# cboin1996/avddpg

Hardware: NVIDIA B200
Metric: platoon-vehicle env-steps/s (higher is better)
Workload: dtype fp16

## Files before the change

### avddpg_b200/csrc/avd_fused3.cu

```cuda
#include <cudaTypedefs.h>

#include <algorithm>

#include "avd_common.cuh"
#include "avd_ddpg_layout.cuh"
#include "avd_umma.cuh"

namespace avd {
namespace fused3 {

using namespace umma;
typedef __nv_bfloat16 bf16;

constexpr int TILE_M = 128, L2N = 128, KB = 64, MAX_KB = 5, L1N = 256;
constexpr int NCONS = 16;
constexpr int NUM_THREADS = 32 * (1 + NCONS);
constexpr int SLOT_BYTES = TILE_M * KB * 2;
constexpr int MAX_SLOT = 7;
constexpr int OFF_W = 0;
constexpr int OFF_RING = OFF_W + MAX_KB * SLOT_BYTES;
constexpr int OFF_DZ = OFF_RING + 5 * SLOT_BYTES;
constexpr int OFF_B1 = OFF_RING + MAX_SLOT * SLOT_BYTES;
constexpr int B1_BYTES = 2 * L1N * 16;
constexpr int OFF_X = OFF_B1 + B1_BYTES;
constexpr int X_BYTES = 2 * TILE_M * 16;
constexpr int OFF_TAB = OFF_X + 2 * X_BYTES;
constexpr int TAB_BYTES = 2048;
constexpr int OFF_PART = OFF_TAB + TAB_BYTES;
constexpr int OFF_BAR = OFF_PART + 2 * 4 * TILE_M * 4;
constexpr int SMEM_BYTES = OFF_BAR + 512 + 1024;
constexpr int kVRows = 49, kVStride = 132, kVBrk = 64;
static_assert((kVRows * kVStride + kVBrk) * 4 + 2 * 4 * TILE_M * 4 <= 2 * SLOT_BYTES, "V table + partial sums exceed the dz2-tile slots");
static_assert(SMEM_BYTES <= 232448, "exceeds the 227 KB shared memory of an sm_100 CTA");

enum Mode { MODE_ACTOR_OUT = 0, MODE_TARGET = 1, MODE_Q = 2, MODE_CRITIC_BWD = 3, MODE_ACTOR_BWD = 4, MODE_CRITIC_ACTION = 5, MODE_ACTOR_SAVE = 6 };

struct Args {
    avd_net_dims d;
    int A;
    int64_t R;
    const float* params;
    int64_t pstride;
    const float* b2f;
    const float* s;
    int64_t s_rs, s_cs;
    const float* act;
    const float* rew;
    float gamma, high;
    const float* y;
    const float* dpi;
    float* out;
    uint32_t* mask_out;
    int mask_words;
    uint32_t* mask2_out;
    float* dact_out;
    const float* vtab;
    float dm_scale;
    float* sdq;
    float* loss;
    int tiles_per_agent, ctas_per_agent;
};

__device__ __forceinline__ uint32_t pack_bf16x2(float a, float b) {
    __nv_bfloat162 v = __floats2bfloat162_rn(a, b);
    return *reinterpret_cast<uint32_t*>(&v);
}
__device__ __forceinline__ uint32_t pack_f16x2(float a, float b) {
    __half2 v = __floats2half2_rn(a, b);
    return *reinterpret_cast<uint32_t*>(&v);
}
__device__ __forceinline__ uint64_t make_desc_noswz(uint32_t saddr, uint32_t lbo_bytes, uint32_t sbo_bytes) {
    return (uint64_t)((saddr & 0x3FFFFu) >> 4) | ((uint64_t)((lbo_bytes >> 4) & 0x3FFFu) << 16) |
           ((uint64_t)((sbo_bytes >> 4) & 0x3FFFu) << 32) | (1ull << 46);
}
__device__ __forceinline__ void split_bf16(float v, bf16& hi, bf16& lo) {
    hi = __float2bfloat16_rn(v);
    lo = __float2bfloat16_rn(v - __bfloat162float(hi));
}
__device__ __forceinline__ uint32_t pack2(bf16 a, bf16 b) {
    return (uint32_t)__bfloat16_as_ushort(a) | ((uint32_t)__bfloat16_as_ushort(b) << 16);
}

template <int MODE, bool F16>
__global__ void __launch_bounds__(NUM_THREADS, 1) fused3_kernel(const __grid_constant__ CUtensorMap tmW, const __grid_constant__ CUtensorMap tmDZ, Args g) {
    constexpr bool CRITIC = MODE != MODE_ACTOR_OUT && MODE != MODE_ACTOR_BWD && MODE != MODE_ACTOR_SAVE;
    constexpr bool SAVE = MODE == MODE_ACTOR_SAVE;
    constexpr bool BWD = MODE == MODE_CRITIC_BWD || MODE == MODE_ACTOR_BWD;
    constexpr bool ACTION = MODE == MODE_CRITIC_ACTION;
    constexpr bool HAS_DZ = BWD;
    constexpr int NKB = CRITIC ? 5 : 4;
    constexpr int NSLOT = (HAS_DZ || ACTION) ? 5 : MAX_SLOT;
    constexpr uint32_t FOP = F16 ? FMT_F16 : FMT_BF16;

    extern __shared__ uint8_t smem_raw[];
    uint8_t* smem = smem_raw + ((1024u - (smem_u32(smem_raw) & 1023u)) & 1023u);
    float* b2f_tab = reinterpret_cast<float*>(smem + OFF_TAB);
    float* w3f_tab = b2f_tab + L2N;
    float* wa_tab = w3f_tab + L2N;
    float* ba_tab = wa_tab + 64;
    float* scal = ba_tab + 64;
    float* part = reinterpret_cast<float*>(smem + OFF_PART);
    uint64_t* a_full = reinterpret_cast<uint64_t*>(smem + OFF_BAR);
    uint64_t* a_empty = a_full + MAX_SLOT;
    uint64_t* acc_full = a_empty + MAX_SLOT;
    uint64_t* acc_empty = acc_full + 2;
    uint64_t* part_full = acc_empty + 2;
    uint64_t* x_full = part_full + 2;
    uint64_t* z1_full = x_full + 2;
    uint64_t* z1_empty = z1_full + 1;
    uint64_t* dz_full = z1_empty + 1;
    uint64_t* dz_empty = dz_full + 1;
    uint64_t* dra_full = dz_empty + 1;
    uint64_t* dra_empty = dra_full + 1;
    uint64_t* w_full = dra_empty + 1;
    uint32_t* tmem_slot = reinterpret_cast<uint32_t*>(w_full + 1);

    const int warp = threadIdx.x >> 5, lane = threadIdx.x & 31;
    const avd_net_dims d = g.d;
    const int la = CRITIC ? d.la : 0;
    const int agent = (int)blockIdx.x / g.ctas_per_agent;
    const int cta = (int)blockIdx.x - agent * g.ctas_per_agent;
    const int T = (g.tiles_per_agent - cta + g.ctas_per_agent - 1) / g.ctas_per_agent;
    const float* P = g.params + (int64_t)agent * g.pstride;

    if (threadIdx.x == 0) {
        tma_prefetch_desc(&tmW);
        if (BWD) tma_prefetch_desc(&tmDZ);
        for (int i = 0; i < MAX_SLOT; ++i) { mbar_init(&a_full[i], 8); mbar_init(&a_empty[i], 1); }
        for (int i = 0; i < 2; ++i) {
            mbar_init(&acc_full[i], 1); mbar_init(&acc_empty[i], NCONS);
            mbar_init(&part_full[i], NCONS); mbar_init(&x_full[i], 4);
        }
        mbar_init(z1_full, 1); mbar_init(z1_empty, NCONS);
        mbar_init(dz_full, NCONS); mbar_init(dz_empty, 1);
        mbar_init(dra_full, 1); mbar_init(dra_empty, 4);
        mbar_init(w_full, 1);
        fence_barrier_init();
    }
    if (warp == 0) tmem_alloc(tmem_slot, 512);

    if (warp >= 1) {
        const int ct = threadIdx.x - 32;
        int64_t oW, ob, og2, obe2, omu2, ovar2, oW3, ob3;
        if (CRITIC) { const CriticOff o = critic_off(d); oW = o.Ws; ob = o.bs; og2 = o.g2; obe2 = o.be2; omu2 = o.mu2; ovar2 = o.var2; oW3 = o.W3; ob3 = o.b3; }
        else { const ActorOff o = actor_off(d); oW = o.W1; ob = o.b1; og2 = o.g2; obe2 = o.be2; omu2 = o.mu2; ovar2 = o.var2; oW3 = o.W3; ob3 = o.b3; }
        if (ct < L1N) {
            bf16 whi[4], wlo[4], bhi, blo;
#pragma unroll
            for (int k = 0; k < 4; ++k) split_bf16(k < d.ns ? P[oW + (int64_t)k * d.l1 + ct] : 0.0f, whi[k], wlo[k]);
            split_bf16(P[ob + ct], bhi, blo);
            const bf16 zero = __float2bfloat16_rn(0.0f);
            const uint4 c0 = make_uint4(pack2(whi[0], whi[1]), pack2(whi[2], whi[3]), pack2(bhi, whi[0]), pack2(whi[1], whi[2]));
            const uint4 c1 = make_uint4(pack2(whi[3], bhi), pack2(wlo[0], wlo[1]), pack2(wlo[2], wlo[3]), pack2(blo, zero));
            *reinterpret_cast<uint4*>(smem + OFF_B1 + ct * 16) = c0;
            *reinterpret_cast<uint4*>(smem + OFF_B1 + L1N * 16 + ct * 16) = c1;
        } else if (ct < L1N + L2N) {
            const int c = ct - L1N;
            const float sc2 = P[og2 + c] / sqrtf(P[ovar2 + c] + kBnEps);
            const float sh2 = P[obe2 + c] - P[omu2 + c] * sc2;
            const float w3 = P[oW3 + c];
            w3f_tab[c] = w3 * sc2;
            const float t = warp_sum(sh2 * w3);
            if (lane == 0) scal[1 + (c >> 5)] = t;
            if (c == 0) scal[5] = P[ob3];
        } else if (ct < L1N + L2N + 64) {
            const int c = ct - L1N - L2N;
            float wa = 0.f, ba = 0.f;
            if (CRITIC && c < d.la) { const CriticOff o = critic_off(d); wa = P[o.Wa + c]; ba = P[o.ba + c]; }
            wa_tab[c] = wa;
            ba_tab[c] = ba;
        }
        fence_proxy_async();
    }
    tc_fence_before();
    __syncthreads();
    tc_fence_after();
    const uint32_t tmem_base = *tmem_slot;
    pdl_wait();
    pdl_launch_dependents();
    if (threadIdx.x >= 32 && threadIdx.x < 32 + L2N) b2f_tab[threadIdx.x - 32] = g.b2f[(int64_t)agent * L2N + threadIdx.x - 32];
    float* vtab_s = reinterpret_cast<float*>(smem + OFF_DZ);
    float* vbrk_s = vtab_s + kVRows * kVStride;
    float* part2 = vbrk_s + kVBrk;
    if (ACTION) {
        const float4* src = reinterpret_cast<const float4*>(g.vtab + (int64_t)agent * (kVRows * kVStride + kVBrk));
        for (int i = threadIdx.x; i < (kVRows * kVStride + kVBrk) / 4; i += NUM_THREADS) reinterpret_cast<float4*>(vtab_s)[i] = src[i];
    }
    __syncthreads();
    const float b3f = scal[5] + scal[1] + scal[2] + scal[3] + scal[4];
    if (T <= 0) {
        __syncthreads();
        if (warp == 0) tmem_dealloc(tmem_base, 512);
        return;
    }

    auto tile_of = [&](int tc) { return cta + tc * g.ctas_per_agent; };

    if (warp == 0) {
        {
            const uint32_t leader = elect_one();
            constexpr uint32_t idesc1 = make_idesc_bf16(TILE_M, L2N, false, false);
            constexpr uint32_t idesc = make_idesc_f16kind(TILE_M, L2N, false, false, FOP, FOP);
            const int F = L1N + la;
            const uint64_t dW = make_smem_desc(smem_u32(smem + OFF_W), 16, 1024);
            const uint64_t dR = make_smem_desc(smem_u32(smem + OFF_RING), 16, 1024);
            const uint64_t dX = make_desc_noswz(smem_u32(smem + OFF_X), TILE_M * 16, 128);
            const uint64_t dB1 = make_desc_noswz(smem_u32(smem + OFF_B1), L1N * 16, 128);
            mbar_expect_tx_p(leader, w_full, (uint32_t)NKB * SLOT_BYTES);
            for (int kb = 0; kb < NKB; ++kb) tma_load_3d_p(leader, smem + OFF_W + kb * SLOT_BYTES, &tmW, w_full, kb * KB, 0, agent);

            auto mma1 = [&](int t) {
                mbar_wait(&x_full[t & 1], ((uint32_t)t >> 1) & 1);
                if (t >= 1) mbar_wait(z1_empty, (uint32_t)(t - 1) & 1);
                tc_fence_after();
#pragma unroll
                for (int h = 0; h < 2; ++h)
                    mma_bf16_p(leader, tmem_base + 256u + (uint32_t)(h * L2N), desc_add(dX, (uint32_t)(t & 1) * X_BYTES), desc_add(dB1, h * (L2N * 16)), idesc1, 0);
                mma_commit_p(leader, z1_full);
            };
            auto mma2 = [&](int t) {
                mbar_wait(&acc_empty[t & 1], (((uint32_t)t >> 1) & 1) ^ 1);
                tc_fence_after();
                const uint32_t tacc = tmem_base + (uint32_t)((t & 1) * L2N);
#pragma unroll
                for (int kb = 0; kb < NKB; ++kb) {
                    const uint32_t kc = (uint32_t)(t * NKB + kb), sl = kc % NSLOT;
                    mbar_wait(&a_full[sl], (kc / NSLOT) & 1);
                    tc_fence_after();
                    const int nm = min(4, (F - kb * KB) / 16);
#pragma unroll
                    for (int j = 0; j < 4; ++j)
                        if (j < nm)
                            mma_bf16_p(leader, tacc, desc_add(dR, sl * SLOT_BYTES + j * 32), desc_add(dW, kb * SLOT_BYTES + j * 32), idesc, (kb | j) != 0);
                    mma_commit_p(leader, &a_empty[sl]);
                }
                mma_commit_p(leader, &acc_full[t & 1]);
            };
            auto dz_out = [&](int t) {
                mbar_wait(dz_full, (uint32_t)t & 1);
                tc_fence_after();
                tma_store_3d_p(leader, &tmDZ, smem + OFF_DZ, 0, tile_of(t) * TILE_M, agent);
                tma_store_3d_p(leader, &tmDZ, smem + OFF_DZ + SLOT_BYTES, KB, tile_of(t) * TILE_M, agent);
                if (leader) {
                    bulk_commit();
                    bulk_wait_read0();
                }
                __syncwarp();
                mbar_arrive_p(leader, dz_empty);
            };

            mbar_wait(w_full, 0);
            {
                mma1(0);
                if (T > 1) mma1(1);
                mma2(0);
                for (int i = 0; i < T; ++i) {
                    if (i + 1 < T) {
                        if (i + 2 < T) mma1(i + 2);
                        mma2(i + 1);
                    }
                    if (BWD && i >= 1) dz_out(i - 1);
                }
                if (BWD) dz_out(T - 1);
            }
        }
    } else {
        const int cw = warp - 1;
        const int q = warp & 3;
        const int c4 = cw >> 2;
        const int row = q * 32 + lane;
        const uint32_t tlane = (uint32_t)(q * 32) << 16;
        const float invR = 1.0f / (float)g.R;
        float sdq_acc = 0.0f, loss_acc = 0.0f;
        uint32_t zneg = 0u;

        auto rowinfo = [&](int tc, bool& valid) -> int64_t {
            const int64_t r_in = (int64_t)tile_of(tc) * TILE_M + row;
            valid = r_in < g.R;
            return (int64_t)agent * g.R + (valid ? r_in : g.R - 1);
        };
        float xs[4] = {0.f, 0.f, 0.f, 0.f}, a_pf = 0.0f, y_pf = 0.0f, a_ag = 0.0f;
        auto xg_of = [&](int tc) { return CRITIC ? 2 * (1 - (tc & 1)) : (tc & 3); };
        auto is_action_quarter = [&](int tc) { return CRITIC && (c4 >> 1) == (tc & 1); };
        auto load_x = [&](int t) {
            bool valid;
            const int64_t n = rowinfo(t, valid);
#pragma unroll
            for (int k = 0; k < 4; ++k) xs[k] = k < d.ns ? __ldg(g.s + n * g.s_rs + k * g.s_cs) : 0.0f;
        };
        auto write_x = [&](int t) {
            bf16 hi[5], lo[5];
#pragma unroll
            for (int k = 0; k < 4; ++k) split_bf16(xs[k], hi[k], lo[k]);
            hi[4] = __float2bfloat16_rn(1.0f);
            lo[4] = __float2bfloat16_rn(0.0f);
            uint8_t* xbase = smem + OFF_X + (t & 1) * X_BYTES;
            *reinterpret_cast<uint4*>(xbase + row * 16) = make_uint4(pack2(hi[0], hi[1]), pack2(hi[2], hi[3]), pack2(hi[4], lo[0]), pack2(lo[1], lo[2]));
            *reinterpret_cast<uint4*>(xbase + TILE_M * 16 + row * 16) =
                make_uint4(pack2(lo[3], lo[4]), pack2(hi[0], hi[1]), pack2(hi[2], hi[3]), pack2(hi[4], lo[4]));
            fence_proxy_async();
            __syncwarp();
            if (lane == 0) mbar_arrive(&x_full[t & 1]);
        };

        auto convert = [&](int tc) {
            bool valid;
            const int64_t nrow = rowinfo(tc, valid);
            const int ga0 = CRITIC ? 2 * (tc & 1) : -1;
            const float a_val = a_pf;
            mbar_wait(z1_full, (uint32_t)tc & 1);
            tc_fence_after();
            const uint32_t kc = (uint32_t)(tc * NKB + c4), sl = kc % NSLOT;
            mbar_wait(&a_empty[sl], ((kc / NSLOT) & 1) ^ 1);
            uint8_t* slot = smem + OFF_RING + sl * SLOT_BYTES + row * 128;
            uint32_t neg[2];
#pragma unroll
            for (int h = 0; h < 2; ++h) {
                float z[32];
                tmem_ld32(tmem_base + 256u + (uint32_t)(c4 * 64 + h * 32) + tlane, z);
                uint32_t m = 0;
                if (BWD || SAVE) {
#pragma unroll
                    for (int j = 0; j < 32; ++j) m = __funnelshift_l(__float_as_uint(z[j]), m, 1);
                }
                neg[h] = m;
#pragma unroll
                for (int k = 0; k < 4; ++k) {
                    const uint4 pk = make_uint4(pack_relu_x2<F16>(z[8 * k], z[8 * k + 1]), pack_relu_x2<F16>(z[8 * k + 2], z[8 * k + 3]),
                                                pack_relu_x2<F16>(z[8 * k + 4], z[8 * k + 5]), pack_relu_x2<F16>(z[8 * k + 6], z[8 * k + 7]));
                    *reinterpret_cast<uint4*>(slot + (((h * 4 + k) ^ (row & 7)) << 4)) = pk;
                }
            }
            tc_fence_before();
            fence_proxy_async();
            __syncwarp();
            if (lane == 0) { mbar_arrive(z1_empty); mbar_arrive_cnt(&a_full[sl], 2); }
            if ((BWD || SAVE) && valid) *reinterpret_cast<uint2*>(g.mask_out + nrow * g.mask_words + 2 * c4) = make_uint2(neg[0], neg[1]);
            if (CRITIC && (c4 == ga0 || c4 == ga0 + 1)) {
                const int j0 = (c4 == ga0) ? 0 : 32;
                const uint32_t kca = (uint32_t)(tc * NKB + 4), sla = kca % NSLOT;
                mbar_wait(&a_empty[sla], ((kca / NSLOT) & 1) ^ 1);
                uint8_t* aslot = smem + OFF_RING + sla * SLOT_BYTES + row * 128;
                float z[32];
                uint32_t m = 0;
#pragma unroll
                for (int j = 0; j < 32; ++j) {
                    z[j] = fmaf(a_val, wa_tab[j0 + j], ba_tab[j0 + j]);
                    if (BWD) m = __funnelshift_l(__float_as_uint(z[j]), m, 1);
                }
#pragma unroll
                for (int k = 0; k < 4; ++k) {
                    const int col = j0 + 8 * k;
                    if (col < la) {
                        const uint4 pk = make_uint4(pack_relu_x2<F16>(z[8 * k], z[8 * k + 1]), pack_relu_x2<F16>(z[8 * k + 2], z[8 * k + 3]),
                                                    pack_relu_x2<F16>(z[8 * k + 4], z[8 * k + 5]), pack_relu_x2<F16>(z[8 * k + 6], z[8 * k + 7]));
                        *reinterpret_cast<uint4*>(aslot + (((col >> 3) ^ (row & 7)) << 4)) = pk;
                    }
                }
                fence_proxy_async();
                __syncwarp();
                if (lane == 0) mbar_arrive(&a_full[sla]);
                if (BWD && valid) g.mask_out[nrow * g.mask_words + 8 + (j0 >> 5)] = m;
            }
            if (c4 == xg_of(tc) && tc + 2 < T) write_x(tc + 2);
            if (tc + 3 < T && c4 == xg_of(tc + 1)) load_x(tc + 3);
            if (tc + 1 < T && is_action_quarter(tc + 1)) {
                bool v1;
                a_pf = __ldg(g.act + rowinfo(tc + 1, v1));
            }
        };

        auto pass1 = [&](int tc) {
            const int buf = tc & 1;
            if (MODE == MODE_TARGET || BWD) {
                bool v0;
                const int64_t n0 = rowinfo(tc, v0);
                if (MODE == MODE_TARGET) { if (c4 == 0) y_pf = __ldg(g.rew + n0); }
                else if (MODE == MODE_CRITIC_BWD) y_pf = __ldg(g.y + n0);
                else y_pf = __ldg(g.dpi + n0);
            }
            const float* vrow = vtab_s;
            if (ACTION) {
                const float a_cur = a_ag;
                if (tc + 1 < T) {
                    bool v1;
                    a_ag = __ldg(g.act + rowinfo(tc + 1, v1));
                }
                int k = 0;
#pragma unroll
                for (int st = 32; st >= 1; st >>= 1)
                    if (vbrk_s[k + st - 1] < a_cur) k += st;
                vrow = vtab_s + k * kVStride + c4 * 32;
            }
            mbar_wait(&acc_full[buf], ((uint32_t)tc >> 1) & 1);
            tc_fence_after();
            float v[32];
            tmem_ld32(tmem_base + (uint32_t)(buf * L2N + c4 * 32) + tlane, v);
            float acc = 0.0f, gacc = 0.0f;
            uint32_t m = 0u;
#pragma unroll
            for (int j = 0; j < 32; j += 4) {
                const float4 b4 = *reinterpret_cast<const float4*>(b2f_tab + c4 * 32 + j);
                const float4 w4 = *reinterpret_cast<const float4*>(w3f_tab + c4 * 32 + j);
                const float t0 = v[j] + b4.x, t1 = v[j + 1] + b4.y, t2 = v[j + 2] + b4.z, t3 = v[j + 3] + b4.w;
                if (ACTION) {
                    const float4 V4 = *reinterpret_cast<const float4*>(vrow + j);
                    gacc += __uint_as_float(__float_as_uint(V4.x) & ~(uint32_t)((int32_t)__float_as_uint(t0) >> 31));
                    gacc += __uint_as_float(__float_as_uint(V4.y) & ~(uint32_t)((int32_t)__float_as_uint(t1) >> 31));
                    gacc += __uint_as_float(__float_as_uint(V4.z) & ~(uint32_t)((int32_t)__float_as_uint(t2) >> 31));
                    gacc += __uint_as_float(__float_as_uint(V4.w) & ~(uint32_t)((int32_t)__float_as_uint(t3) >> 31));
                }
                acc = fmaf(fmaxf(t0, 0.0f), w4.x, acc);
                acc = fmaf(fmaxf(t1, 0.0f), w4.y, acc);
                acc = fmaf(fmaxf(t2, 0.0f), w4.z, acc);
                acc = fmaf(fmaxf(t3, 0.0f), w4.w, acc);
                if (HAS_DZ || SAVE) {
                    m = __funnelshift_l(__float_as_uint(t0), m, 1);
                    m = __funnelshift_l(__float_as_uint(t1), m, 1);
                    m = __funnelshift_l(__float_as_uint(t2), m, 1);
                    m = __funnelshift_l(__float_as_uint(t3), m, 1);
                }
            }
            if (HAS_DZ) zneg = m;
            if (SAVE) {
                bool v1;
                const int64_t n1 = rowinfo(tc, v1);
                if (v1) g.mask2_out[n1 * 4 + c4] = m;
            }
            part[(buf * 4 + c4) * TILE_M + row] = acc;
            if (ACTION) part2[(buf * 4 + c4) * TILE_M + row] = gacc;
            tc_fence_before();
            __syncwarp();
            if (lane == 0) {
                if (HAS_DZ || c4 != 0) mbar_arrive(&acc_empty[buf]);
                mbar_arrive(&part_full[buf]);
            }
        };

        auto pass2 = [&](int tc) {
            const int buf = tc & 1;
            if (!HAS_DZ && c4 != 0) return;
            bool valid;
            const int64_t nrow = rowinfo(tc, valid);
            const float yv = y_pf;
            mbar_wait(&part_full[buf], ((uint32_t)tc >> 1) & 1);
            const float* pb = part + buf * 4 * TILE_M + row;
            const float qv = pb[0] + pb[TILE_M] + pb[2 * TILE_M] + pb[3 * TILE_M] + b3f;
            if (!HAS_DZ) {
                float o;
                if (MODE == MODE_ACTOR_OUT || SAVE) {
                    const float t = tanhf(qv);
                    o = g.high * t;
                    if (SAVE && valid) g.dact_out[nrow] = g.high * (1.0f - t * t);
                }
                else if (MODE == MODE_TARGET) o = yv + g.gamma * qv;
                else if (ACTION) {
                    const float* pg = part2 + buf * 4 * TILE_M + row;
                    o = -invR * (pg[0] + pg[TILE_M] + pg[2 * TILE_M] + pg[3 * TILE_M]);
                    if (valid) loss_acc -= qv * invR;
                }
                else o = qv;
                if (valid) g.out[nrow] = o;
                __syncwarp();
                if (lane == 0) mbar_arrive(&acc_empty[buf]);
                return;
            }
            float dq = 0.0f;
            if (MODE == MODE_CRITIC_BWD) {
                const float diff = qv - yv;
                dq = valid ? 2.0f * diff * invR : 0.0f;
                if (c4 == 0) {
                    if (valid) loss_acc = fmaf(diff, diff * invR, loss_acc);
                    if (valid && g.out) g.out[nrow] = qv;
                }
            } else if (MODE == MODE_ACTOR_BWD) {
                const float t = tanhf(qv);
                dq = valid ? yv * g.high * (1.0f - t * t) : 0.0f;
            }
            if (c4 == 0) sdq_acc += dq;
            float v[32];
            {
                const float dqs = dq * g.dm_scale;
#pragma unroll
                for (int j = 0; j < 32; ++j) v[j] = (zneg & (0x80000000u >> j)) ? 0.0f : dqs;
            }
            mbar_wait(dz_empty, ((uint32_t)tc & 1) ^ 1);
            uint8_t* dzrow = smem + OFF_DZ + (c4 >> 1) * SLOT_BYTES + row * 128;
#pragma unroll
            for (int k = 0; k < 4; ++k) {
                const uint4 pk = make_uint4(pack_x2<F16>(v[8 * k], v[8 * k + 1]), pack_x2<F16>(v[8 * k + 2], v[8 * k + 3]),
                                            pack_x2<F16>(v[8 * k + 4], v[8 * k + 5]), pack_x2<F16>(v[8 * k + 6], v[8 * k + 7]));
                *reinterpret_cast<uint4*>(dzrow + ((((c4 & 1) * 4 + k) ^ (row & 7)) << 4)) = pk;
            }
            fence_proxy_async();
            __syncwarp();
            if (lane == 0) mbar_arrive(dz_full);
        };

        if (cw < 4) { load_x(0); write_x(0); }
        else if (cw < 8 && T > 1) { load_x(1); write_x(1); }
        if (T > 2 && c4 == xg_of(0)) load_x(2);
        if (is_action_quarter(0)) {
            bool v0;
            a_pf = __ldg(g.act + rowinfo(0, v0));
        }
        if (ACTION) {
            bool v0;
            a_ag = __ldg(g.act + rowinfo(0, v0));
        }
        convert(0);
        for (int i = 0; i < T; ++i) {
            {
                if (i + 1 < T) convert(i + 1);
                if (i >= 1) pass2(i - 1);
                pass1(i);
            }
        }
        pass2(T - 1);

        if ((HAS_DZ || ACTION) && c4 == 0) {
            const float sl = warp_sum(loss_acc), sd = warp_sum(sdq_acc);
            if (lane == 0) {
                if (g.loss && MODE != MODE_ACTOR_BWD) atomicAdd(g.loss + 2 * agent + (MODE == MODE_CRITIC_BWD ? 0 : 1), sl);
                if (BWD) atomicAdd(g.sdq + agent, sd);
            }
        }
    }
    tc_fence_before();
    __syncthreads();
    if (warp == 0) {
        tc_fence_after();
        tmem_dealloc(tmem_base, 512);
    }
}

static PFN_cuTensorMapEncodeTiled encode_fn() {
    static PFN_cuTensorMapEncodeTiled fn = nullptr;
    if (!fn) {
        void* p = nullptr;
        cudaDriverEntryPointQueryResult q;
        if (cudaGetDriverEntryPoint("cuTensorMapEncodeTiled", &p, cudaEnableDefault, &q) == cudaSuccess && q == cudaDriverEntryPointSuccess)
            fn = reinterpret_cast<PFN_cuTensorMapEncodeTiled>(p);
    }
    return fn;
}

static int make_map(CUtensorMap* tm, const void* base, uint64_t inner, uint64_t rows, uint64_t batch, uint64_t pitch, uint64_t batch_stride) {
    PFN_cuTensorMapEncodeTiled enc = encode_fn();
    if (!enc) {
        set_error("cuTensorMapEncodeTiled is not available from the driver");
        return AVD_ERR_CUDA;
    }
    cuuint64_t dims[3] = {inner, rows, batch};
    cuuint64_t strides[2] = {pitch * 2, batch_stride * 2};
    cuuint32_t box[3] = {KB, TILE_M, 1};
    cuuint32_t estr[3] = {1, 1, 1};
    CUresult r = enc(tm, CU_TENSOR_MAP_DATA_TYPE_BFLOAT16, 3, const_cast<void*>(base), dims, strides, box, estr, CU_TENSOR_MAP_INTERLEAVE_NONE,
                     CU_TENSOR_MAP_SWIZZLE_128B, CU_TENSOR_MAP_L2_PROMOTION_L2_256B, CU_TENSOR_MAP_FLOAT_OOB_FILL_NONE);
    if (r != CUDA_SUCCESS) {
        set_error("cuTensorMapEncodeTiled failed with %d (inner=%llu rows=%llu batch=%llu pitch=%llu)", (int)r, (unsigned long long)inner,
                  (unsigned long long)rows, (unsigned long long)batch, (unsigned long long)pitch);
        return AVD_ERR_CUDA;
    }
    return AVD_OK;
}

bool supported(const avd_net_dims& d) {
    return d.l2 == L2N && d.ns >= 1 && d.ns <= 4 && d.l1 == L1N && d.la % 16 == 0 && d.la >= 16 && d.la < kVRows;
}
int vtab_rows() { return kVRows; }
int vtab_stride() { return kVStride; }
int vtab_floats() { return kVRows * kVStride + kVBrk; }

template <int MODE, bool F16>
static int launch2(const CUtensorMap& tmW, const CUtensorMap& tmDZ, const Args& g, dim3 grid, cudaStream_t st) {
    static bool attr_set = false;
    if (!attr_set) {
        AVD_CUDA_OK(cudaFuncSetAttribute(fused3_kernel<MODE, F16>, cudaFuncAttributeMaxDynamicSharedMemorySize, SMEM_BYTES));
        attr_set = true;
    }
    AVD_CUDA_OK(launch_pdl(fused3_kernel<MODE, F16>, dim3(grid), dim3(NUM_THREADS), SMEM_BYTES, st, tmW, tmDZ, g));
    AVD_LAUNCH_OK();
    return AVD_OK;
}
template <int MODE>
static int launch(bool f16, const CUtensorMap& tmW, const CUtensorMap& tmDZ, const Args& g, dim3 grid, cudaStream_t st) {
    return f16 ? launch2<MODE, true>(tmW, tmDZ, g, grid, st) : launch2<MODE, false>(tmW, tmDZ, g, grid, st);
}

int run(int mode, bool f16, const avd_net_dims& d, int A, int64_t R, const float* params, int64_t pstride, const bf16* W2T, const float* b2f,
        const float* vtab, const float* s, int64_t s_rs, int64_t s_cs, const float* act, const float* rew, float gamma, float high, const float* y,
        const float* dpi, float* out, uint32_t* mask_out, bf16* DZ_out, float dm_scale, float* sdq, float* loss, cudaStream_t st,
        uint32_t* mask2_out, float* dact_out) {
    if (!supported(d)) {
        set_error("fused pass kernel does not support these layer sizes");
        return AVD_ERR_UNSUPPORTED;
    }
    const bool critic = mode != MODE_ACTOR_OUT && mode != MODE_ACTOR_BWD && mode != MODE_ACTOR_SAVE;
    const bool bwd = mode == MODE_CRITIC_BWD || mode == MODE_ACTOR_BWD;
    const int F = critic ? d.l1 + d.la : d.l1;
    AVD_REQUIRE(params && W2T && b2f && s, "null buffer");
    AVD_REQUIRE(A >= 1 && R >= 1 && R < (int64_t)1 << 31, "rows per agent must fit the 32-bit TMA coordinates");
    AVD_REQUIRE(!critic || act, "critic passes need actions");
    AVD_REQUIRE(!bwd || (mask_out && DZ_out && sdq), "backward passes need mask / dz2 / sdq outputs");
    AVD_REQUIRE(mode != MODE_CRITIC_ACTION || (vtab && d.la < kVRows), "the critic-action pass needs its V table (la <= %d)", kVRows - 1);
    AVD_REQUIRE(bwd || out, "null output");
    AVD_REQUIRE(mode != MODE_ACTOR_SAVE || (mask_out && mask2_out && dact_out), "MODE_ACTOR_SAVE needs the mask / d(action) outputs");
    CUtensorMap tmW, tmDZ;
    if (int rc = make_map(&tmW, W2T, (uint64_t)F, L2N, (uint64_t)A, (uint64_t)F, (uint64_t)F * L2N)) return rc;
    tmDZ = tmW;
    if (bwd)
        if (int rc = make_map(&tmDZ, DZ_out, L2N, (uint64_t)R, (uint64_t)A, L2N, (uint64_t)R * L2N)) return rc;
    Args g;
    g.d = d; g.A = A; g.R = R; g.params = params; g.pstride = pstride; g.b2f = b2f; g.s = s; g.s_rs = s_rs; g.s_cs = s_cs; g.act = act;
    g.rew = rew; g.gamma = gamma; g.high = high; g.y = y; g.dpi = dpi; g.out = out; g.mask_out = mask_out; g.mask_words = 2 * ((F + KB - 1) / KB);
    g.vtab = vtab; g.dm_scale = dm_scale; g.sdq = sdq; g.loss = loss; g.mask2_out = mask2_out; g.dact_out = dact_out;
    g.tiles_per_agent = (int)((R + TILE_M - 1) / TILE_M);
    g.ctas_per_agent = std::max(1, std::min(g.tiles_per_agent, sm_count() / std::max(1, A)));
    const dim3 grid((unsigned)(g.ctas_per_agent * A));
    switch (mode) {
        case MODE_ACTOR_OUT: return launch<MODE_ACTOR_OUT>(f16, tmW, tmDZ, g, grid, st);
        case MODE_TARGET: return launch<MODE_TARGET>(f16, tmW, tmDZ, g, grid, st);
        case MODE_Q: return launch<MODE_Q>(f16, tmW, tmDZ, g, grid, st);
        case MODE_CRITIC_BWD: return launch<MODE_CRITIC_BWD>(f16, tmW, tmDZ, g, grid, st);
        case MODE_ACTOR_BWD: return launch<MODE_ACTOR_BWD>(f16, tmW, tmDZ, g, grid, st);
        case MODE_CRITIC_ACTION: return launch<MODE_CRITIC_ACTION>(f16, tmW, tmDZ, g, grid, st);
        case MODE_ACTOR_SAVE: return launch<MODE_ACTOR_SAVE>(f16, tmW, tmDZ, g, grid, st);
    }
    set_error("unknown fused pass mode %d", mode);
    return AVD_ERR_INVALID_ARG;
}

}
}
```

Baseline: 15.58 million.

## Fold layer-2 bias into MMA, use incremental ring slots and packed FMA epilogue

Adds a bias-seeding MMA that writes the layer-2 bias into the TMEM accumulator using a ones column times a 3-way bf16 split of the bias, so the epilogue no longer reads and adds b2f per element. Replaces the per-iteration modulo slot/phase arithmetic with running slot/phase counters in both producer and consumer warps. Replaces the 64-bit rowinfo index math with 32-bit row offsets and precomputed per-agent base pointers. Rewrites the epilogue reductions with packed float2 FFMA2/FADD2 instructions. This adds one extra small MMA per tile and bias precision becomes limited to a three-term bf16 split, in exchange for less epilogue ALU and index work.

```diff
diff --git a/avddpg_b200/csrc/avd_fused3.cu b/avddpg_b200/csrc/avd_fused3.cu
--- a/avddpg_b200/csrc/avd_fused3.cu
+++ b/avddpg_b200/csrc/avd_fused3.cu
@@ -24,7 +24,9 @@
 constexpr int B1_BYTES = 2 * L1N * 16;
 constexpr int OFF_X = OFF_B1 + B1_BYTES;
 constexpr int X_BYTES = 2 * TILE_M * 16;
-constexpr int OFF_TAB = OFF_X + 2 * X_BYTES;
+constexpr int OFF_BIAS = OFF_X + 2 * X_BYTES;
+constexpr int BIAS_BYTES = 2 * TILE_M * 16;
+constexpr int OFF_TAB = OFF_BIAS + 2 * BIAS_BYTES;
 constexpr int TAB_BYTES = 2048;
 constexpr int OFF_PART = OFF_TAB + TAB_BYTES;
 constexpr int OFF_BAR = OFF_PART + 2 * 4 * TILE_M * 4;
@@ -94,8 +96,7 @@
 
     extern __shared__ uint8_t smem_raw[];
     uint8_t* smem = smem_raw + ((1024u - (smem_u32(smem_raw) & 1023u)) & 1023u);
-    float* b2f_tab = reinterpret_cast<float*>(smem + OFF_TAB);
-    float* w3f_tab = b2f_tab + L2N;
+    float* w3f_tab = reinterpret_cast<float*>(smem + OFF_TAB);
     float* wa_tab = w3f_tab + L2N;
     float* ba_tab = wa_tab + 64;
     float* scal = ba_tab + 64;
@@ -170,6 +171,12 @@
             wa_tab[c] = wa;
             ba_tab[c] = ba;
         }
+        if (ct < TILE_M) {
+            const uint32_t one = __bfloat16_as_ushort(__float2bfloat16_rn(1.0f));
+            *reinterpret_cast<uint4*>(smem + OFF_BIAS + ct * 16) = make_uint4(one | (one << 16), one, 0u, 0u);
+            *reinterpret_cast<uint4*>(smem + OFF_BIAS + TILE_M * 16 + ct * 16) = make_uint4(0u, 0u, 0u, 0u);
+            *reinterpret_cast<uint4*>(smem + OFF_BIAS + BIAS_BYTES + L2N * 16 + ct * 16) = make_uint4(0u, 0u, 0u, 0u);
+        }
         fence_proxy_async();
     }
     tc_fence_before();
@@ -178,7 +185,15 @@
     const uint32_t tmem_base = *tmem_slot;
     pdl_wait();
     pdl_launch_dependents();
-    if (threadIdx.x >= 32 && threadIdx.x < 32 + L2N) b2f_tab[threadIdx.x - 32] = g.b2f[(int64_t)agent * L2N + threadIdx.x - 32];
+    if (threadIdx.x >= 32 && threadIdx.x < 32 + L2N) {
+        const int c = threadIdx.x - 32;
+        const float b = g.b2f[(int64_t)agent * L2N + c];
+        bf16 hi, mid, lo, unused;
+        split_bf16(b, hi, mid);
+        split_bf16(b - __bfloat162float(hi) - __bfloat162float(mid), lo, unused);
+        *reinterpret_cast<uint4*>(smem + OFF_BIAS + BIAS_BYTES + c * 16) = make_uint4(pack2(hi, mid), pack2(lo, __float2bfloat16_rn(0.0f)), 0u, 0u);
+        fence_proxy_async();
+    }
     float* vtab_s = reinterpret_cast<float*>(smem + OFF_DZ);
     float* vbrk_s = vtab_s + kVRows * kVStride;
     float* part2 = vbrk_s + kVBrk;
@@ -206,6 +221,9 @@
             const uint64_t dR = make_smem_desc(smem_u32(smem + OFF_RING), 16, 1024);
             const uint64_t dX = make_desc_noswz(smem_u32(smem + OFF_X), TILE_M * 16, 128);
             const uint64_t dB1 = make_desc_noswz(smem_u32(smem + OFF_B1), L1N * 16, 128);
+            const uint64_t dBiasA = make_desc_noswz(smem_u32(smem + OFF_BIAS), TILE_M * 16, 128);
+            const uint64_t dBiasB = make_desc_noswz(smem_u32(smem + OFF_BIAS + BIAS_BYTES), L2N * 16, 128);
+            uint32_t slot = 0, phase = 0;
             mbar_expect_tx_p(leader, w_full, (uint32_t)NKB * SLOT_BYTES);
             for (int kb = 0; kb < NKB; ++kb) tma_load_3d_p(leader, smem + OFF_W + kb * SLOT_BYTES, &tmW, w_full, kb * KB, 0, agent);
 
@@ -222,17 +240,18 @@
                 mbar_wait(&acc_empty[t & 1], (((uint32_t)t >> 1) & 1) ^ 1);
                 tc_fence_after();
                 const uint32_t tacc = tmem_base + (uint32_t)((t & 1) * L2N);
+                mma_bf16_p(leader, tacc, dBiasA, dBiasB, idesc1, 0);
 #pragma unroll
                 for (int kb = 0; kb < NKB; ++kb) {
-                    const uint32_t kc = (uint32_t)(t * NKB + kb), sl = kc % NSLOT;
-                    mbar_wait(&a_full[sl], (kc / NSLOT) & 1);
+                    mbar_wait(&a_full[slot], phase);
                     tc_fence_after();
                     const int nm = min(4, (F - kb * KB) / 16);
 #pragma unroll
                     for (int j = 0; j < 4; ++j)
                         if (j < nm)
-                            mma_bf16_p(leader, tacc, desc_add(dR, sl * SLOT_BYTES + j * 32), desc_add(dW, kb * SLOT_BYTES + j * 32), idesc, (kb | j) != 0);
-                    mma_commit_p(leader, &a_empty[sl]);
+                            mma_bf16_p(leader, tacc, desc_add(dR, slot * SLOT_BYTES + j * 32), desc_add(dW, kb * SLOT_BYTES + j * 32), idesc, 1);
+                    mma_commit_p(leader, &a_empty[slot]);
+                    if (++slot == NSLOT) { slot = 0; phase ^= 1; }
                 }
                 mma_commit_p(leader, &acc_full[t & 1]);
             };
@@ -274,19 +293,22 @@
         float sdq_acc = 0.0f, loss_acc = 0.0f;
         uint32_t zneg = 0u;
 
-        auto rowinfo = [&](int tc, bool& valid) -> int64_t {
-            const int64_t r_in = (int64_t)tile_of(tc) * TILE_M + row;
-            valid = r_in < g.R;
-            return (int64_t)agent * g.R + (valid ? r_in : g.R - 1);
-        };
+        const uint32_t R32 = (uint32_t)g.R;
+        const uint32_t row0 = (uint32_t)(cta * TILE_M + row), row_step = (uint32_t)(g.ctas_per_agent * TILE_M);
+        auto row_of = [&](int tc) { return row0 + (uint32_t)tc * row_step; };
+        auto ld_row = [&](uint32_t r) { return min(r, R32 - 1); };
+        const int64_t agent_row = (int64_t)agent * g.R;
+        const float* s_a = g.s + agent_row * g.s_rs;
+        const float* act_a = CRITIC ? g.act + agent_row : nullptr;
+        uint32_t* mask_a = (BWD || SAVE) ? g.mask_out + agent_row * g.mask_words : nullptr;
+        uint32_t cslot = (uint32_t)c4, cphase = 0, aslot = 4, aphase = 0;
         float xs[4] = {0.f, 0.f, 0.f, 0.f}, a_pf = 0.0f, y_pf = 0.0f, a_ag = 0.0f;
         auto xg_of = [&](int tc) { return CRITIC ? 2 * (1 - (tc & 1)) : (tc & 3); };
         auto is_action_quarter = [&](int tc) { return CRITIC && (c4 >> 1) == (tc & 1); };
         auto load_x = [&](int t) {
-            bool valid;
-            const int64_t n = rowinfo(t, valid);
-#pragma unroll
-            for (int k = 0; k < 4; ++k) xs[k] = k < d.ns ? __ldg(g.s + n * g.s_rs + k * g.s_cs) : 0.0f;
+            const float* sp = s_a + (int64_t)ld_row(row_of(t)) * g.s_rs;
+#pragma unroll
+            for (int k = 0; k < 4; ++k) xs[k] = k < d.ns ? __ldg(sp + k * g.s_cs) : 0.0f;
         };
         auto write_x = [&](int t) {
             bf16 hi[5], lo[5];
@@ -304,14 +326,16 @@
         };
 
         auto convert = [&](int tc) {
-            bool valid;
-            const int64_t nrow = rowinfo(tc, valid);
+            const uint32_t r = row_of(tc);
+            const bool valid = r < R32;
             const int ga0 = CRITIC ? 2 * (tc & 1) : -1;
             const float a_val = a_pf;
             mbar_wait(z1_full, (uint32_t)tc & 1);
             tc_fence_after();
-            const uint32_t kc = (uint32_t)(tc * NKB + c4), sl = kc % NSLOT;
-            mbar_wait(&a_empty[sl], ((kc / NSLOT) & 1) ^ 1);
+            const uint32_t sl = cslot;
+            mbar_wait(&a_empty[sl], cphase ^ 1);
+            cslot += NKB;
+            if (cslot >= NSLOT) { cslot -= NSLOT; cphase ^= 1; }
             uint8_t* slot = smem + OFF_RING + sl * SLOT_BYTES + row * 128;
             uint32_t neg[2];
 #pragma unroll
@@ -335,11 +359,16 @@
             fence_proxy_async();
             __syncwarp();
             if (lane == 0) { mbar_arrive(z1_empty); mbar_arrive_cnt(&a_full[sl], 2); }
-            if ((BWD || SAVE) && valid) *reinterpret_cast<uint2*>(g.mask_out + nrow * g.mask_words + 2 * c4) = make_uint2(neg[0], neg[1]);
+            uint32_t* mrow = (BWD || SAVE) ? mask_a + (uint64_t)r * g.mask_words : nullptr;
+            if ((BWD || SAVE) && valid) *reinterpret_cast<uint2*>(mrow + 2 * c4) = make_uint2(neg[0], neg[1]);
+            const uint32_t sla = aslot, pha = aphase;
+            if (CRITIC) {
+                aslot += NKB;
+                if (aslot >= NSLOT) { aslot -= NSLOT; aphase ^= 1; }
+            }
             if (CRITIC && (c4 == ga0 || c4 == ga0 + 1)) {
                 const int j0 = (c4 == ga0) ? 0 : 32;
-                const uint32_t kca = (uint32_t)(tc * NKB + 4), sla = kca % NSLOT;
-                mbar_wait(&a_empty[sla], ((kca / NSLOT) & 1) ^ 1);
+                mbar_wait(&a_empty[sla], pha ^ 1);
                 uint8_t* aslot = smem + OFF_RING + sla * SLOT_BYTES + row * 128;
                 float z[32];
                 uint32_t m = 0;
@@ -360,32 +389,26 @@
                 fence_proxy_async();
                 __syncwarp();
                 if (lane == 0) mbar_arrive(&a_full[sla]);
-                if (BWD && valid) g.mask_out[nrow * g.mask_words + 8 + (j0 >> 5)] = m;
+                if (BWD && valid) mrow[8 + (j0 >> 5)] = m;
             }
             if (c4 == xg_of(tc) && tc + 2 < T) write_x(tc + 2);
             if (tc + 3 < T && c4 == xg_of(tc + 1)) load_x(tc + 3);
-            if (tc + 1 < T && is_action_quarter(tc + 1)) {
-                bool v1;
-                a_pf = __ldg(g.act + rowinfo(tc + 1, v1));
-            }
+            if (tc + 1 < T && is_action_quarter(tc + 1)) a_pf = __ldg(act_a + ld_row(row_of(tc + 1)));
         };
 
         auto pass1 = [&](int tc) {
             const int buf = tc & 1;
+            const uint32_t r = row_of(tc);
             if (MODE == MODE_TARGET || BWD) {
-                bool v0;
-                const int64_t n0 = rowinfo(tc, v0);
-                if (MODE == MODE_TARGET) { if (c4 == 0) y_pf = __ldg(g.rew + n0); }
-                else if (MODE == MODE_CRITIC_BWD) y_pf = __ldg(g.y + n0);
-                else y_pf = __ldg(g.dpi + n0);
+                const uint32_t n0 = ld_row(r);
+                if (MODE == MODE_TARGET) { if (c4 == 0) y_pf = __ldg(g.rew + agent_row + n0); }
+                else if (MODE == MODE_CRITIC_BWD) y_pf = __ldg(g.y + agent_row + n0);
+                else y_pf = __ldg(g.dpi + agent_row + n0);
             }
             const float* vrow = vtab_s;
             if (ACTION) {
                 const float a_cur = a_ag;
-                if (tc + 1 < T) {
-                    bool v1;
-                    a_ag = __ldg(g.act + rowinfo(tc + 1, v1));
-                }
+                if (tc + 1 < T) a_ag = __ldg(act_a + ld_row(row_of(tc + 1)));
                 int k = 0;
 #pragma unroll
                 for (int st = 32; st >= 1; st >>= 1)
@@ -394,41 +417,30 @@
             }
             mbar_wait(&acc_full[buf], ((uint32_t)tc >> 1) & 1);
             tc_fence_after();
-            float v[32];
-            tmem_ld32(tmem_base + (uint32_t)(buf * L2N + c4 * 32) + tlane, v);
-            float acc = 0.0f, gacc = 0.0f;
+            float t[32];
+            tmem_ld32(tmem_base + (uint32_t)(buf * L2N + c4 * 32) + tlane, t);
+            float2 acc = make_float2(0.0f, 0.0f), gacc = make_float2(0.0f, 0.0f);
             uint32_t m = 0u;
+            auto vsel = [](float V, float z) { return __uint_as_float(__float_as_uint(V) & ~(uint32_t)((int32_t)__float_as_uint(z) >> 31)); };
 #pragma unroll
             for (int j = 0; j < 32; j += 4) {
-                const float4 b4 = *reinterpret_cast<const float4*>(b2f_tab + c4 * 32 + j);
                 const float4 w4 = *reinterpret_cast<const float4*>(w3f_tab + c4 * 32 + j);
-                const float t0 = v[j] + b4.x, t1 = v[j + 1] + b4.y, t2 = v[j + 2] + b4.z, t3 = v[j + 3] + b4.w;
                 if (ACTION) {
                     const float4 V4 = *reinterpret_cast<const float4*>(vrow + j);
-                    gacc += __uint_as_float(__float_as_uint(V4.x) & ~(uint32_t)((int32_t)__float_as_uint(t0) >> 31));
-                    gacc += __uint_as_float(__float_as_uint(V4.y) & ~(uint32_t)((int32_t)__float_as_uint(t1) >> 31));
-                    gacc += __uint_as_float(__float_as_uint(V4.z) & ~(uint32_t)((int32_t)__float_as_uint(t2) >> 31));
-                    gacc += __uint_as_float(__float_as_uint(V4.w) & ~(uint32_t)((int32_t)__float_as_uint(t3) >> 31));
-                }
-                acc = fmaf(fmaxf(t0, 0.0f), w4.x, acc);
-                acc = fmaf(fmaxf(t1, 0.0f), w4.y, acc);
-                acc = fmaf(fmaxf(t2, 0.0f), w4.z, acc);
-                acc = fmaf(fmaxf(t3, 0.0f), w4.w, acc);
+                    gacc = __fadd2_rn(make_float2(vsel(V4.x, t[j]), vsel(V4.y, t[j + 1])), gacc);
+                    gacc = __fadd2_rn(make_float2(vsel(V4.z, t[j + 2]), vsel(V4.w, t[j + 3])), gacc);
+                }
+                acc = __ffma2_rn(make_float2(fmaxf(t[j], 0.0f), fmaxf(t[j + 1], 0.0f)), make_float2(w4.x, w4.y), acc);
+                acc = __ffma2_rn(make_float2(fmaxf(t[j + 2], 0.0f), fmaxf(t[j + 3], 0.0f)), make_float2(w4.z, w4.w), acc);
                 if (HAS_DZ || SAVE) {
-                    m = __funnelshift_l(__float_as_uint(t0), m, 1);
-                    m = __funnelshift_l(__float_as_uint(t1), m, 1);
-                    m = __funnelshift_l(__float_as_uint(t2), m, 1);
-                    m = __funnelshift_l(__float_as_uint(t3), m, 1);
+#pragma unroll
+                    for (int i = 0; i < 4; ++i) m = __funnelshift_l(__float_as_uint(t[j + i]), m, 1);
                 }
             }
             if (HAS_DZ) zneg = m;
-            if (SAVE) {
-                bool v1;
-                const int64_t n1 = rowinfo(tc, v1);
-                if (v1) g.mask2_out[n1 * 4 + c4] = m;
-            }
-            part[(buf * 4 + c4) * TILE_M + row] = acc;
-            if (ACTION) part2[(buf * 4 + c4) * TILE_M + row] = gacc;
+            if (SAVE && r < R32) g.mask2_out[(uint64_t)(agent_row + r) * 4 + c4] = m;
+            part[(buf * 4 + c4) * TILE_M + row] = acc.x + acc.y;
+            if (ACTION) part2[(buf * 4 + c4) * TILE_M + row] = gacc.x + gacc.y;
             tc_fence_before();
             __syncwarp();
             if (lane == 0) {
@@ -440,8 +452,9 @@
         auto pass2 = [&](int tc) {
             const int buf = tc & 1;
             if (!HAS_DZ && c4 != 0) return;
-            bool valid;
-            const int64_t nrow = rowinfo(tc, valid);
+            const uint32_t r = row_of(tc);
+            const bool valid = r < R32;
+            const int64_t nrow = agent_row + r;
             const float yv = y_pf;
             mbar_wait(&part_full[buf], ((uint32_t)tc >> 1) & 1);
             const float* pb = part + buf * 4 * TILE_M + row;
@@ -500,14 +513,8 @@
         if (cw < 4) { load_x(0); write_x(0); }
         else if (cw < 8 && T > 1) { load_x(1); write_x(1); }
         if (T > 2 && c4 == xg_of(0)) load_x(2);
-        if (is_action_quarter(0)) {
-            bool v0;
-            a_pf = __ldg(g.act + rowinfo(0, v0));
-        }
-        if (ACTION) {
-            bool v0;
-            a_ag = __ldg(g.act + rowinfo(0, v0));
-        }
+        if (is_action_quarter(0)) a_pf = __ldg(act_a + ld_row(row_of(0)));
+        if (ACTION) a_ag = __ldg(act_a + ld_row(row_of(0)));
         convert(0);
         for (int i = 0; i < T; ++i) {
             {
```

New measurement: 16.03 million, median of 6. 1.03x the previous value.
